# nrsyed/pytorch-yolov3

Hardware: AMD Instinct MI355X
Metric: frames/sec (608x608) (higher is better)
Workload: dtype bf16

## Files before the change

### include/yolov3_hip.h

```cpp
#ifndef YOLOV3_HIP_H
#define YOLOV3_HIP_H

#include <stddef.h>
#include <stdint.h>

#ifdef __cplusplus
extern "C" {
#endif

#define Y3_ABI_VERSION 6

#define Y3_OK 0
#define Y3_ERR_INVALID (-1)
#define Y3_ERR_HIP (-2)
#define Y3_ERR_NODEVICE (-3)

#define Y3_F32 0
#define Y3_BF16 1
#define Y3_F16 2
#define Y3_F64 3

#define Y3_OP_CONV 1
#define Y3_OP_MAXPOOL 2
#define Y3_OP_UPSAMPLE 3
// ... 28 lines not shown
  const float *d_bias;
  int32_t n_anchor, n_attr;
  float anchor_w[8], anchor_h[8];
  int32_t row_offset, rows_total;
  float net_w, net_h;
  float *d_bbox;
  float *d_prob;
  int64_t *d_cls;
  int32_t block_idx;
  int32_t reserved;
  const void *d_weight_frag;
} y3_op;

typedef struct y3_plan y3_plan;

#define Y3_AM_HALO_WIDE 0x0001u
#define Y3_AM_IGEMM3_MID 0x0002u
#define Y3_AM_HALO_NARROW 0x0004u
#define Y3_AM_IGEMM3_1X1_DEEP 0x0008u
#define Y3_AM_HALO_MID 0x0010u
#define Y3_AM_IGEMM3_NARROW 0x0020u
#define Y3_AM_IGEMM3_1X1_BM64 0x0040u
#define Y3_AM_PATCH_WIDE 0x0080u
#define Y3_AM_HALO_TILE256 0x0200u
#define Y3_AM_NO_BN_SHRINK 0x0400u
#define Y3_AM_NO_SMALL_GRID 0x0800u
#define Y3_AM_NO_WRES 0x1000u
#define Y3_AM_HALO_DW 0x4000u
#define Y3_AM_HALO_DW_ALWAYS 0x8000u
#define Y3_AM_1X1_DW 0x10000u
#define Y3_AM_SMALL_DW 0x20000u
#define Y3_AM_SMALL_DW_ALWAYS 0x40000u
#define Y3_AM_SMALL_DW_WIDE 0x80000u
#define Y3_AM_WRES_ALWAYS 0x2000u
#define Y3_AM_DEFAULT (Y3_AM_HALO_WIDE | Y3_AM_HALO_NARROW | Y3_AM_IGEMM3_1X1_DEEP | Y3_AM_HALO_MID | Y3_AM_PATCH_WIDE | Y3_AM_HALO_DW | Y3_AM_1X1_DW | Y3_AM_SMALL_DW | Y3_AM_SMALL_DW_WIDE)
#define Y3_AM_IGEMM_ONLY 0u

typedef struct y3_options {
  int32_t auto_mask, unused0, igemm_version, igemm_ns, igemm_bm;
  int32_t use_graph, fuse_stem, fuse_head, fuse_spp, decode_lanes;
  int32_t fuse_block;
  int32_t reserved[5];
} y3_options;

int y3_abi_version(void);
const char *y3_last_error(void);
int y3_device_count(void);

int y3_plan_create(const y3_op *ops, int n_ops, const void *d_zero, y3_plan **out_plan);
int y3_plan_create_ex(const y3_op *ops, int n_ops, const void *d_zero, const y3_options *options, y3_plan **out_plan);
void y3_options_default(y3_options *options);
void y3_plan_destroy(y3_plan *plan);
int y3_plan_run(y3_plan *plan, const void *d_input, void *stream);
int y3_plan_run_timed(y3_plan *plan, const void *d_input, void *stream, float *ms_per_op);
int y3_plan_run_profiled(y3_plan *plan, const void *d_input, void *stream, float *kernel_ms_per_op);
const char *y3_plan_op_kernel(const y3_plan *plan, int op_index);
double y3_plan_op_flops(const y3_plan *plan, int op_index);
double y3_plan_op_bytes(const y3_plan *plan, int op_index);

int y3_conv_path(const y3_op *op);

size_t y3_conv_fragment_weight_bytes(const y3_op *op, const y3_options *options);
int y3_conv_make_fragment_weights(const y3_op *op, void *d_dst, void *stream);

int y3_set_tuning(const char *key, int value);

int y3_op_run(const y3_op *op, const void *d_input, const void *d_zero, void *stream);

// ... 32 lines not shown
```

### pytorch-yolov3_amd/csrc/api.hip

```cpp
#include <stdarg.h>
#include <string.h>

#include <atomic>
#include <new>
#include <vector>

#include "common.h"

static_assert(sizeof(y3_op) == 248, "y3_op layout is part of the ABI (ctypes mirror in yolov3/_hip.py)");

namespace {
thread_local char g_err[512] = "";
}

static y3_options g_y3_defaults = { (int32_t)Y3_AM_DEFAULT,  0,  2,  2,
                                    0,  0,  1,  1,  1,
                                    4,  0, {0, 0, 0, 0, 0}};
static thread_local const y3_options *tl_y3_opt = nullptr;
const y3_options &y3_opt() { return tl_y3_opt ? *tl_y3_opt : g_y3_defaults; }
static thread_local Y3KernelTimer *tl_y3_timer = nullptr;
Y3KernelTimer *y3_kernel_timer() { return tl_y3_timer; }
#if defined(Y3_X_NOEPI) || defined(Y3_X_S2BOUND) || defined(Y3_X_DEBUG) || defined(Y3_STAMPS)
#define Y3_HAS_DEBUG_KEY 1
static int g_y3_debug = 0;
// ... 75 lines not shown
            const unsigned am = (unsigned)y3_opt().auto_mask;
            const int w = op.in_w;
            const bool k3 = op.ksize == 3 && op.stride == 1 && op.in_c >= 128 && op.out_c >= 128 && !(op.flags & Y3_F_OUT_F32);
            const bool halo_ok = k3 && y3_conv_halo_ws_fits(op);
            bool want_halo = false, want_ws = false;
            if (k3 && w > 64) want_halo = am & Y3_AM_HALO_WIDE;
            else if (k3 && w > 32) { want_halo = am & Y3_AM_HALO_MID; want_ws = am & Y3_AM_IGEMM3_MID; }
            else if (k3) { want_halo = am & Y3_AM_HALO_NARROW; want_ws = am & Y3_AM_IGEMM3_NARROW; }
            else if (op.ksize == 1 && op.in_c >= 1024 && op.out_c >= 128 && !(op.flags & Y3_F_OUT_F32))
              want_ws = (am & Y3_AM_IGEMM3_1X1_DEEP) &&
                        ((am & Y3_AM_NO_SMALL_GRID) || (long long)y3_ceil_div(op.batch * op.out_h * op.out_w, 128) * y3_ceil_div(op.out_c, 128) >= y3_device_cus() / 4);
            if ((am & Y3_AM_1X1_DW) && y3_conv1x1_dw_pays(op))
              return y3_launch_conv1x1_dw(op, in, d_zero, s, name, dry_run, frag_w ? frag_w : op.d_weight_frag);
            const bool small_dw = (am & (Y3_AM_SMALL_DW | Y3_AM_SMALL_DW_ALWAYS)) && !(am & Y3_AM_NO_SMALL_GRID);
            if (small_dw && (y3_conv_dw48_fits(op) || (op.ksize == 3 && y3_conv_dw48_fits_wide(op))))
              return y3_launch_conv_dw48(op, in, d_zero, s, name, dry_run, frag_w ? frag_w : op.d_weight_frag);
            if (!(am & Y3_AM_NO_WRES) && y3_conv1x1_wres_supported(op) && ((am & Y3_AM_WRES_ALWAYS) || y3_conv1x1_wres_pays(op)))
              return y3_launch_conv1x1_wres(op, in, d_zero, s, name, dry_run);
            if (small_dw && op.ksize == 1 && y3_conv_dw48_fits_wide(op))
              return y3_launch_conv_dw48(op, in, d_zero, s, name, dry_run, frag_w ? frag_w : op.d_weight_frag);
            if ((am & Y3_AM_IGEMM3_1X1_BM64) && op.ksize == 1 && op.in_c >= 256 && op.out_c >= 128 && !(op.flags & Y3_F_OUT_F32) &&
                y3_is16(op.dtype))
              return y3_launch_conv_igemm(op, in, d_zero, s, name, dry_run, 3, 3, 64);
            if ((am & Y3_AM_PATCH_WIDE) && op.ksize == 3 && op.stride == 1 && w > 128 && op.out_c >= 128 && y3_conv_patch_fits(op))
              return y3_launch_conv_patch(op, in, d_zero, s, name, dry_run);
            const long long halo_tiles = (long long)y3_ceil_div(op.batch * op.in_h * op.in_w, 192) * (op.out_c / 128);
            const bool small_grid = !(am & Y3_AM_NO_SMALL_GRID) && k3 && halo_tiles < (3 * y3_device_cus()) / 4;
            if (k3 && !small_grid && halo_ok && (((am & Y3_AM_HALO_DW) && y3_conv_halo_dw_pays(op)) ||
                                                 ((am & Y3_AM_HALO_DW_ALWAYS) && y3_conv_halo_dw_fits(op))))
              return y3_launch_conv_halo_dw(op, in, d_zero, s, name, dry_run, frag_w ? frag_w : op.d_weight_frag);
            if (small_grid && y3_is16(op.dtype)) return y3_launch_conv_igemm(op, in, d_zero, s, name, dry_run, 3, 3);
            if (want_halo && halo_ok && !small_grid) return y3_launch_conv_halo(op, in, d_zero, s, name, dry_run);
            if (want_ws) return y3_launch_conv_igemm(op, in, d_zero, s, name, dry_run, 3, 3);
            if (!(am & Y3_AM_NO_SMALL_GRID) && op.ksize == 3 && op.stride == 2 && op.out_c >= 128 && y3_is16(op.dtype) && !(op.flags & Y3_F_OUT_F32) &&
                ((op.in_c == 256 && (long long)op.batch * op.out_h * op.out_w >= 16384) ||
                 (op.in_c == 64 && (long long)op.batch * op.out_h * op.out_w <= 49152)))
              return y3_launch_conv_igemm(op, in, d_zero, s, name, dry_run, 3, 3);
          }
          return y3_launch_conv_igemm(op, in, d_zero, s, name, dry_run);
        }
        case 1: return y3_launch_conv_small(op, in, s, name, dry_run);
        case 3: return y3_launch_conv_stem_mfma(op, in, s, name, dry_run);
        default: return y3_launch_conv_direct(op, in, s, name, dry_run);
      }
    }
    case Y3_OP_MAXPOOL: return y3_launch_maxpool(op, in, s, name, dry_run);
    case Y3_OP_UPSAMPLE: return y3_launch_upsample(op, in, s, name, dry_run);
    case Y3_OP_ADD: return y3_launch_add(op, in, s, name, dry_run);
    case Y3_OP_COPY: return y3_launch_copy(op, in, s, name, dry_run);
    case Y3_OP_YOLO: return y3_launch_yolo(op, in, s, name, dry_run);
    default: break;
  }
  y3_set_error("op for block %d: unknown kind %d", op.block_idx, op.kind);
  return Y3_ERR_INVALID;
}

int run_op(y3_plan *plan, size_t i, const void *d_input, hipStream_t s, const char **name) {
  if (plan->fuse[i] == 2) return Y3_OK;
  if (plan->fuse[i] == 3) return y3_launch_conv_fused_resblock(plan->ops[i], plan->ops[i + 1], s, name, false);
  if (plan->fuse[i] == 6) return y3_launch_conv_block_fused(plan->ops[i], plan->ops[i + 1], s, name, false);
  if (plan->fuse[i] == 4) return y3_launch_conv_head_decode(plan->ops[i], plan->ops[i + 1], plan->d_zero, s, name, false, plan->frag_w[i]);
  if (plan->fuse[i] == 5) return y3_launch_maxpool_spp(plan->ops[i], plan->ops[i + 1], plan->ops[i + 2], s, name, false);
  if (plan->fuse[i] == 1) {
    const y3_op &op0 = plan->ops[i];
    const void *in = (op0.flags & Y3_F_PLAN_INPUT) ? d_input : op0.d_in;
    Y3_REQUIRE(in != nullptr, "op for block %d has no input pointer", op0.block_idx);
    return y3_launch_conv_fused_stem_s2(op0, plan->ops[i + 1], in, s, name, false);
  }
  return dispatch(plan->ops[i], d_input, plan->d_zero, s, name, false, plan->frag_w[i]);
}

bool uses_fragment_weights(const char *kernel) {
  return strncmp(kernel, "conv_halo_dw_", 13) == 0 || strncmp(kernel, "conv1x1_dw_", 11) == 0 || strncmp(kernel, "conv_dw48_", 10) == 0 ||
         strncmp(kernel, "conv_head_decode_dw_", 20) == 0;
}

int make_private_fragment_weights(y3_plan *p, size_t i) {
  const y3_op &op = p->ops[i];
  int prev = -1, owner = -1;
  Y3_HIP_CHECK(hipGetDevice(&prev));
  hipPointerAttribute_t attr;
  if (op.d_weight && hipPointerGetAttributes(&attr, op.d_weight) == hipSuccess) owner = attr.device;
  else (void)hipGetLastError();
  if (owner >= 0 && owner != prev) Y3_HIP_CHECK(hipSetDevice(owner));
  int rc = Y3_OK;
  void *w = nullptr;
  hipStream_t s = nullptr;
  do {
    if (hipMalloc(&w, y3_conv_halo_dw_weight_bytes(op)) != hipSuccess) {
      (void)hipGetLastError();
      y3_set_error("y3_plan_create: no memory for the fragment-order weights of block %d", op.block_idx);
      rc = Y3_ERR_HIP;
      break;
    }
    p->frag_w[i] = w;
    p->frag_own[i] = 1;
    if (hipStreamCreateWithFlags(&s, hipStreamNonBlocking) != hipSuccess) { s = nullptr; rc = Y3_ERR_HIP; }
    if (rc == Y3_OK) rc = y3_conv_halo_dw_make_weights(op, w, s);
    if (rc == Y3_OK && hipStreamSynchronize(s) != hipSuccess) rc = Y3_ERR_HIP;
    if (rc == Y3_ERR_HIP) y3_set_error("y3_plan_create: fragment-order weights of block %d: %s", op.block_idx, hipGetErrorString(hipGetLastError()));
  } while (0);
  if (s) (void)hipStreamDestroy(s);
  if (owner >= 0 && owner != prev) (void)hipSetDevice(prev);
  return rc;
}

}
// ... 2 lines not shown

int y3_abi_version(void) { return Y3_ABI_VERSION; }

const char *y3_last_error(void) { return g_err; }

int y3_device_count(void) {
  int n = 0;
  if (hipGetDeviceCount(&n) != hipSuccess) return 0;
  int ok = 0;
  for (int i = 0; i < n; ++i) {
    hipDeviceProp_t prop;
    if (hipGetDeviceProperties(&prop, i) == hipSuccess && strncmp(prop.gcnArchName, "gfx950", 6) == 0) ++ok;
  }
  return ok;
}

int y3_conv_path(const y3_op *op) {
  if (!op || op->kind != Y3_OP_CONV) return -1;
  return conv_path(*op);
}

size_t y3_conv_fragment_weight_bytes(const y3_op *op, const y3_options *options) {
  if (!op || op->kind != Y3_OP_CONV || conv_path(*op) != 0) return 0;
  y3_options o = options ? *options : g_y3_defaults;
  OptScope scope(&o);
  const char *name = "";
  if (y3_opt().fuse_head && y3_conv_head_dw_fits(*op)) return y3_conv_halo_dw_weight_bytes(*op);
  if (dispatch(*op, nullptr, nullptr, nullptr, &name, true) != Y3_OK) return 0;
  return uses_fragment_weights(name) ? y3_conv_halo_dw_weight_bytes(*op) : 0;
}

int y3_conv_make_fragment_weights(const y3_op *op, void *d_dst, void *stream) {
  Y3_REQUIRE(op && d_dst && op->d_weight, "y3_conv_make_fragment_weights: bad arguments");
  Y3_REQUIRE(y3_conv_halo_dw_fits(*op) || y3_conv1x1_dw_pays(*op) || y3_conv_dw48_fits(*op) || y3_conv_dw48_fits_wide(*op) || y3_conv_head_dw_fits(*op),
             "conv block %d: not a layer of a direct-weights kernel", op->block_idx);
  return y3_conv_halo_dw_make_weights(*op, d_dst, static_cast<hipStream_t>(stream));
}

void y3_options_default(y3_options *options) {
  if (options) *options = g_y3_defaults;
}

int y3_plan_create(const y3_op *ops, int n_ops, const void *d_zero, y3_plan **out_plan) {
  return y3_plan_create_ex(ops, n_ops, d_zero, nullptr, out_plan);
}

int y3_plan_create_ex(const y3_op *ops, int n_ops, const void *d_zero, const y3_options *options, y3_plan **out_plan) {
  Y3_REQUIRE(ops && n_ops > 0 && out_plan, "y3_plan_create: bad arguments");
  Y3_REQUIRE(d_zero, "y3_plan_create: d_zero (zeroed device page) is required");
  y3_plan *p = new (std::nothrow) y3_plan;
  Y3_REQUIRE(p, "y3_plan_create: out of host memory");
  p->opt = options ? *options : g_y3_defaults;
  OptScope scope(&p->opt);
  p->ops.assign(ops, ops + n_ops);
  p->kernel.assign(n_ops, "");
  p->frag_w.assign(n_ops, nullptr);
  p->frag_own.assign(n_ops, 0);
  p->d_zero = d_zero;
  p->fuse.assign(n_ops, 0);
  for (int i = 0; i + 2 < n_ops; ++i)
    if (y3_opt().fuse_spp && y3_maxpool_spp_supported(p->ops[i], p->ops[i + 1], p->ops[i + 2])) {
      p->fuse[i] = 5;
      p->fuse[i + 1] = p->fuse[i + 2] = 2;
    }
  for (int i = 0; i + 1 < n_ops; ++i)
    if (p->fuse[i] != 0) continue;
    else if ((p->ops[i].flags & Y3_F_FUSE_NEXT) && p->ops[i].kind == Y3_OP_CONV &&
        y3_conv_fused_stem_s2_supported(p->ops[i], p->ops[i + 1])) {
// ... 250 lines not shown
```

### pytorch-yolov3_amd/csrc/common.h

```cpp
#pragma once
#include <hip/hip_runtime.h>
#include <hip/hip_ext.h>
#include <stdint.h>
#include <stdio.h>

#include <mutex>

#include "yolov3_hip.h"

typedef __bf16 bf16_t;
typedef float f32x4 __attribute__((ext_vector_type(4)));
typedef float f32x2 __attribute__((ext_vector_type(2)));
typedef __bf16 bf16x8 __attribute__((ext_vector_type(8)));
typedef __bf16 bf16x4 __attribute__((ext_vector_type(4)));
typedef _Float16 f16_t;
typedef _Float16 f16x8 __attribute__((ext_vector_type(8)));
typedef _Float16 f16x4 __attribute__((ext_vector_type(4)));
typedef uint32_t u32x4 __attribute__((ext_vector_type(4)));
typedef uint32_t u32x2 __attribute__((ext_vector_type(2)));

#define Y3_WAVE 64
#ifndef Y3_AUX_W
#define Y3_AUX_W 0
#endif
// ... 64 lines not shown
  }
};

static inline bool y3_is16(int dtype) { return dtype == Y3_BF16 || dtype == Y3_F16; }
static inline int y3_elem_size(int dtype) { return y3_is16(dtype) ? 2 : 4; }
#define Y3_KNAME(dt, pre, post) ((dt) == Y3_BF16 ? pre "bf16" post : ((dt) == Y3_F16 ? pre "f16" post : pre "f32" post))
template <typename F>
static inline int y3_by_dtype(int dtype, F &&f) {
  if (dtype == Y3_BF16) return f(bf16_t{});
  if (dtype == Y3_F16) return f(f16_t{});
  return f(float{});
}
template <typename F>
static inline int y3_by_dtype16(int dtype, F &&f) {
  return dtype == Y3_F16 ? f(f16_t{}) : f(bf16_t{});
}
static inline int y3_ceil_div(int a, int b) { return (a + b - 1) / b; }
static inline void y3_fast_div(uint32_t d, uint32_t &mul, uint32_t &sh) {
  if (d <= 1) { mul = 0; sh = 0; return; }
  sh = 0;
  while ((1u << sh) < d) ++sh;
  mul = (uint32_t)((((uint64_t)1 << 32) * (((uint64_t)1 << sh) - d)) / d + 1);
}

__device__ __forceinline__ int y3_xcd_remap(int bid, int nwg) {
  const int q = nwg >> 3, r = nwg & 7;
  const int xcd = bid & 7, idx = bid >> 3;
  const int base = xcd < r ? xcd * (q + 1) : r * (q + 1) + (xcd - r) * q;
  return base + idx;
}

__host__ __device__ __forceinline__ constexpr int y3_pair_perm(int j) {
  return (j & ~31) | (((j >> 2) & 3) << 3) | (((j >> 4) & 1) << 2) | (j & 3);
}

template <typename T>
__device__ __forceinline__ float y3_to_float(T v);
template <>
__device__ __forceinline__ float y3_to_float<float>(float v) { return v; }
template <>
__device__ __forceinline__ float y3_to_float<bf16_t>(bf16_t v) { return (float)v; }
template <>
__device__ __forceinline__ float y3_to_float<f16_t>(f16_t v) { return (float)v; }

template <typename T>
__device__ __forceinline__ T y3_from_float(float v);
template <>
__device__ __forceinline__ float y3_from_float<float>(float v) { return v; }
template <>
__device__ __forceinline__ bf16_t y3_from_float<bf16_t>(float v) { return (bf16_t)v; }
template <>
__device__ __forceinline__ f16_t y3_from_float<f16_t>(float v) { return (f16_t)v; }

template <typename T>
struct H16;
template <>
struct H16<bf16_t> {
  typedef bf16x8 v8;
  typedef bf16x4 v4;
  static __device__ __forceinline__ f32x4 mfma(const v8 &w, const v8 &x, const f32x4 &acc) {
    return __builtin_amdgcn_mfma_f32_16x16x32_bf16(w, x, acc, 0, 0, 0);
  }
};
template <>
struct H16<f16_t> {
  typedef f16x8 v8;
// ... 153 lines not shown
int y3_launch_conv_fused_stem_s2(const y3_op &op0, const y3_op &op1, const void *d_in, hipStream_t s,
                                 const char **kernel_name, bool dry_run);
bool y3_conv_fused_resblock_supported(const y3_op &op0, const y3_op &op1);
int y3_launch_conv_fused_resblock(const y3_op &op0, const y3_op &op1, hipStream_t s, const char **kernel_name,
                                  bool dry_run);
bool y3_conv_block_fused_supported(const y3_op &op0, const y3_op &op1);
int y3_launch_conv_block_fused(const y3_op &op0, const y3_op &op1, hipStream_t s, const char **kernel_name, bool dry_run);
bool y3_conv_head_decode_supported(const y3_op &op0, const y3_op &op1);
int y3_launch_conv_head_decode(const y3_op &op0, const y3_op &op1, const void *d_zero, hipStream_t s,
                               const char **kernel_name, bool dry_run, const void *frag_w = nullptr);
bool y3_conv_head_dw_fits(const y3_op &op0);
int y3_launch_conv_head_decode_dw(const y3_op &op0, const y3_op &op1, const void *d_zero, hipStream_t s, const char **kernel_name,
                                  bool dry_run, const void *frag_w);
bool y3_conv_halo_ws_fits(const y3_op &op);
bool y3_conv_halo_dw_fits(const y3_op &op);
bool y3_conv_halo_dw_pays(const y3_op &op);
size_t y3_conv_halo_dw_weight_bytes(const y3_op &op);
int y3_conv_halo_dw_make_weights(const y3_op &op, void *dst, hipStream_t s);
int y3_launch_conv_halo_dw(const y3_op &op, const void *d_in, const void *d_zero, hipStream_t s,
                           const char **kernel_name, bool dry_run, const void *frag_w);
int y3_launch_conv_halo(const y3_op &op, const void *d_in, const void *d_zero, hipStream_t s,
                        const char **kernel_name, bool dry_run);
bool y3_conv1x1_wres_supported(const y3_op &op);
bool y3_conv1x1_wres_pays(const y3_op &op);
int y3_launch_conv1x1_wres(const y3_op &op, const void *d_in, const void *d_zero, hipStream_t s, const char **kernel_name,
                           bool dry_run);
bool y3_conv1x1_dw_pays(const y3_op &op);
int y3_launch_conv1x1_dw(const y3_op &op, const void *d_in, const void *d_zero, hipStream_t s, const char **kernel_name,
                         bool dry_run, const void *frag_w);
bool y3_conv_dw48_fits(const y3_op &op);
bool y3_conv_dw48_fits_wide(const y3_op &op);
int y3_launch_conv_dw48(const y3_op &op, const void *d_in, const void *d_zero, hipStream_t s, const char **kernel_name,
                        bool dry_run, const void *frag_w);
bool y3_conv_patch_fits(const y3_op &op);
int y3_launch_conv_patch(const y3_op &op, const void *d_in, const void *d_zero, hipStream_t s,
                         const char **kernel_name, bool dry_run);
const y3_options &y3_opt();
bool y3_conv_igemm_supported(const y3_op &op);
```

### pytorch-yolov3_amd/csrc/conv_dw48.hip

```cpp
#include <utility>

#include "common.h"

namespace {

typedef __attribute__((address_space(3))) void lds_void;
typedef const __attribute__((address_space(1))) void gbl_void;

struct Dw48Args {
  const char *in;
  const char *wgt;
  const float *scale;
  const float *bias;
  const char *res;
  char *out;
  const char *zero;
  int M, H, W, HW, in_ld, out_ld, res_ld, k_ld;
  int in_h, in_w;
  int n_ctiles;
  int nwc;
  int m_tiles;
  int m_inner;
  int hr;
  uint32_t mul_hw, sh_hw, mul_w, sh_w;
// ... 25 lines not shown
  constexpr int SWZ = NKT == 1 ? 7 : 15;
  static_assert((ST == 1 && NH == 1) || (ST == 2 && KS == 3), "stride 2 and channel halves: the 3x3 form only");
  constexpr int BM = 48, MI = 3, NI = 2;
  constexpr int TAPS = KS * KS;
  constexpr int RB = NKT * 128;
  constexpr int S = NKT * TAPS * 2;
  constexpr int DEPTH = S < Y3_DW48_DEPTH ? S : Y3_DW48_DEPTH;
  extern __shared__ __attribute__((aligned(16))) char smem[];

  const int tid = threadIdx.x;
  const int lane = tid & 63;
  const int wave = __builtin_amdgcn_readfirstlane(tid >> 6);
  const int nwaves = blockDim.x >> 6;
  const int fr = lane & 15, fq = lane >> 4;
  const int tile = y3_xcd_remap(blockIdx.x, gridDim.x);
  const int mt = p.m_inner ? tile % p.m_tiles : tile / p.n_ctiles;
  const int ct = p.m_inner ? tile / p.m_tiles : tile % p.n_ctiles;
  const int m0 = mt * BM;
  const int n0 = (ct * p.nwc + wave) * 32;

  const long long q0 = (long long)m0 - (KS == 3 ? p.W + 1 : 0);
  const int pieces = ((p.hr + 1) * RB + 1023) >> 10;
  auto stage = [&](int h) {
    for (int i = wave; i < pieces; i += nwaves) {
      const int o = i * 1024 + lane * 16;
      const int r = o / RB, cpos = (o - r * RB) >> 4;
      const int c = cpos ^ (r & SWZ);
      long long q;
      bool ok;
      if constexpr (ST == 1) {
        q = q0 + r;
        ok = r < p.hr && q >= 0 && q < p.M;
      } else {
        const int e1 = 48, e2 = 97, e3 = 145 + p.W;
        const int pr = r >= e2 ? 1 : 0, pc = ((r >= e1 && r < e2) || r >= e3) ? 1 : 0;
        const int base = r < e1 ? 0 : (r < e2 ? e1 + 1 : (r < e3 ? e2 + p.W : e3 + p.W + 1));
        const long long mm = (long long)m0 + r - base;
        ok = r < p.hr && mm >= 0 && mm < p.M;
        const uint32_t um = ok ? (uint32_t)mm : 0u;
        const uint32_t img = (__umulhi(um, p.mul_hw) + um) >> p.sh_hw;
        const uint32_t rem = um - img * (uint32_t)p.HW;
        const uint32_t oy = (__umulhi(rem, p.mul_w) + rem) >> p.sh_w;
        const uint32_t ox = rem - oy * (uint32_t)p.W;
        q = ((long long)img * p.in_h + 2 * oy + pr) * p.in_w + 2 * ox + pc;
      }
      const char *src = ok ? p.in + (q * p.in_ld) * 2 + h * RB + c * 16 : p.zero;
      __builtin_amdgcn_global_load_lds((gbl_void *)src, (lds_void *)(smem + i * 1024), 16, 0, 0);
    }
  };

  const uint32_t kblocks = (uint32_t)p.k_ld / 32u;
  const uint32_t w_lane = (uint32_t)lane * 16;
  const char *wb[NI];
#pragma unroll
  for (int ni = 0; ni < NI; ++ni) wb[ni] = p.wgt + (((long long)(n0 / 16 + ni) * kblocks) << 10);
  u32x4 wf[DEPTH][NI];
  uint32_t w_img = w_lane;
  if (wave >= p.nwc) {
#pragma unroll 1
    for (int h = 0; h < NH; ++h) {
      if (h > 0) __builtin_amdgcn_s_barrier();
      stage(h);
      asm volatile("s_waitcnt vmcnt(0)" ::: "memory");
      __builtin_amdgcn_s_barrier();
    }
    return;
  }
  stage(0);
  asm volatile("" ::: "memory");
  auto load_w = [&](auto sc, u32x4 (&w)[NI]) {
    constexpr int s = decltype(sc)::value;
    constexpr int kt = s / (2 * TAPS), tap = (s / 2) % TAPS, kh = s & 1;
    const uint32_t voff = w_img + (uint32_t)((tap * (NH * NKT * 2) + kt * 2 + kh) << 10);
    const char *b0 = wb[0], *b1 = wb[1];
    asm volatile("global_load_dwordx4 %0, %1, %2" : "=v"(w[0]) : "v"(voff), "s"(b0));
    asm volatile("global_load_dwordx4 %0, %1, %2" : "=v"(w[1]) : "v"(voff), "s"(b1));
  };
  dw48_for<DEPTH>([&](auto sc) { load_w(sc, wf[decltype(sc)::value]); });

  typedef const __attribute__((address_space(3))) u32x4 lds_u32x4;
  const int lds0 = (int)(size_t)(lds_void *)smem;
  const int zrow = lds0 + p.hr * RB;
  int abase[TAPS][MI], fk4[TAPS];
  {
    uint32_t tapmask[MI];
#pragma unroll
    for (int mi = 0; mi < MI; ++mi) {
      tapmask[mi] = 0x1FFu;
      if constexpr (KS == 3) {
        const uint32_t m = (uint32_t)(m0 + mi * 16 + fr);
        const uint32_t img = (__umulhi(m, p.mul_hw) + m) >> p.sh_hw;
        const uint32_t rem = m - img * (uint32_t)p.HW;
        const uint32_t oy = (__umulhi(rem, p.mul_w) + rem) >> p.sh_w;
        const uint32_t ox = rem - oy * (uint32_t)p.W;
        const uint32_t vx = (ox >= 1u ? 1u : 0u) | 2u | (ST == 2 || ox + 1u < (uint32_t)p.W ? 4u : 0u);
        tapmask[mi] = (oy >= 1u ? vx : 0u) | (vx << 3) | (ST == 2 || oy + 1u < (uint32_t)p.H ? vx << 6 : 0u);
      }
    }
#pragma unroll
    for (int tap = 0; tap < TAPS; ++tap) {
      int r0 = fr + (KS == 3 ? (tap / 3) * p.W + tap % 3 : 0);
      if constexpr (ST == 2) {
        const int ky = tap / 3, kx = tap % 3;
        r0 = fr + (ky == 1 ? (kx == 1 ? 0 : 48) : (kx == 1 ? 97 : 145 + p.W)) + (kx == 2 ? 1 : 0) + (ky == 2 ? p.W : 0);
      }
      fk4[tap] = (fq ^ (r0 & SWZ)) << 4;
#pragma unroll
      for (int mi = 0; mi < MI; ++mi)
        abase[tap][mi] = ((tapmask[mi] >> tap) & 1u) ? lds0 + (mi * 16 + r0) * RB : zrow;
    }
  }

  f32x4 acc[MI][NI];
#pragma unroll
  for (int mi = 0; mi < MI; ++mi)
#pragma unroll
    for (int ni = 0; ni < NI; ++ni) acc[mi][ni] = f32x4{0.f, 0.f, 0.f, 0.f};

  u32x4 xf[3][MI];
  auto read_x = [&](auto sc, u32x4 (&x)[MI]) {
    constexpr int s = decltype(sc)::value;
    constexpr int kt = s / (2 * TAPS), tap = (s / 2) % TAPS, kh = s & 1;
    const int off = ((kt * 8 + kh * 4) << 4) ^ fk4[tap];
#pragma unroll
    for (int mi = 0; mi < MI; ++mi) x[mi] = *reinterpret_cast<lds_u32x4 *>(abase[tap][mi] + off);
  };
  auto mma = [&](const u32x4 (&x)[MI], const u32x4 (&w)[NI]) {
#pragma unroll
    for (int mi = 0; mi < MI; ++mi)
#pragma unroll
      for (int ni = 0; ni < NI; ++ni) acc[mi][ni] = y3_mfma16<T>(w[ni], x[mi], acc[mi][ni]);
  };
  auto run_image = [&]() {
    asm volatile("s_waitcnt vmcnt(%0)" ::"n"(2 * (DEPTH - 1)) : "memory");
    __builtin_amdgcn_s_barrier();
    read_x(HalfC<0>{}, xf[0]);
    if constexpr (S > 1) read_x(HalfC<1>{}, xf[1]);
// ... 202 lines not shown
```

### pytorch-yolov3_amd/yolov3/_hip.py

```python
import ctypes
import os

import torch


_RUNTIME_DEFAULT_QUEUES = 4


def hw_queues():
    try:
        return int(os.environ.get("GPU_MAX_HW_QUEUES") or _RUNTIME_DEFAULT_QUEUES), True
    except ValueError:
        return _RUNTIME_DEFAULT_QUEUES, False

_HERE = os.path.dirname(os.path.abspath(__file__))
LIB_PATH = os.environ.get("Y3_HIP_LIB") or os.path.join(_HERE, "..", "lib", "libyolov3_hip.so")

Y3_F32, Y3_BF16, Y3_F16, Y3_F64 = 0, 1, 2, 3
OP_CONV, OP_MAXPOOL, OP_UPSAMPLE, OP_ADD, OP_COPY, OP_YOLO = 1, 2, 3, 4, 5, 6
F_LEAKY, F_RESIDUAL, F_OUT_F32, F_IN_NCHW_F32, F_IN_NHWC_U8BGR, F_PLAN_INPUT, F_FUSE_NEXT = 1, 2, 4, 8, 16, 32, 64
PATH_IGEMM, PATH_STEM, PATH_DIRECT, PATH_STEM_MFMA = 0, 1, 2, 3


class Y3Op(ctypes.Structure):
    _fields_ = [
        ("kind", ctypes.c_int32), ("dtype", ctypes.c_int32), ("flags", ctypes.c_uint32),
        ("batch", ctypes.c_int32),
        ("in_h", ctypes.c_int32), ("in_w", ctypes.c_int32), ("in_c", ctypes.c_int32), ("in_ld", ctypes.c_int32),
        ("out_h", ctypes.c_int32), ("out_w", ctypes.c_int32), ("out_c", ctypes.c_int32), ("out_ld", ctypes.c_int32),
        ("ksize", ctypes.c_int32), ("stride", ctypes.c_int32), ("pad", ctypes.c_int32),
        ("res_ld", ctypes.c_int32), ("k_ld", ctypes.c_int32), ("cout_pad", ctypes.c_int32),
        ("d_in", ctypes.c_void_p), ("d_out", ctypes.c_void_p), ("d_res", ctypes.c_void_p),
        ("d_weight", ctypes.c_void_p), ("d_scale", ctypes.c_void_p), ("d_bias", ctypes.c_void_p),
        ("n_anchor", ctypes.c_int32), ("n_attr", ctypes.c_int32),
        ("anchor_w", ctypes.c_float * 8), ("anchor_h", ctypes.c_float * 8),
        ("row_offset", ctypes.c_int32), ("rows_total", ctypes.c_int32),
        ("net_w", ctypes.c_float), ("net_h", ctypes.c_float),
        ("d_bbox", ctypes.c_void_p), ("d_prob", ctypes.c_void_p), ("d_cls", ctypes.c_void_p),
        ("block_idx", ctypes.c_int32), ("reserved", ctypes.c_int32),
        ("d_weight_frag", ctypes.c_void_p),
    ]


class Y3Options(ctypes.Structure):
    _fields_ = [(name, ctypes.c_int32) for name in (
        "auto_mask", "unused0", "igemm_version", "igemm_ns", "igemm_bm", "use_graph", "fuse_stem", "fuse_head",
        "fuse_spp", "decode_lanes", "fuse_block")] + [("reserved", ctypes.c_int32 * 5)]


AM_HALO_WIDE, AM_IGEMM3_MID, AM_HALO_NARROW, AM_IGEMM3_1X1_DEEP = 0x0001, 0x0002, 0x0004, 0x0008
AM_HALO_MID, AM_IGEMM3_NARROW, AM_IGEMM3_1X1_BM64, AM_PATCH_WIDE = 0x0010, 0x0020, 0x0040, 0x0080
AM_HALO_TILE256, AM_NO_BN_SHRINK, AM_NO_SMALL_GRID, AM_NO_WRES, AM_WRES_ALWAYS = 0x0200, 0x0400, 0x0800, 0x1000, 0x2000
AM_HALO_DW, AM_HALO_DW_ALWAYS = 0x4000, 0x8000
AM_1X1_DW = 0x10000
AM_SMALL_DW_ALWAYS = 0x40000
AM_SMALL_DW = 0x20000
AM_SMALL_DW_WIDE = 0x80000
AM_DEFAULT = (AM_HALO_WIDE | AM_HALO_NARROW | AM_IGEMM3_1X1_DEEP | AM_HALO_MID | AM_PATCH_WIDE | AM_HALO_DW | AM_1X1_DW | AM_SMALL_DW |
              AM_SMALL_DW_WIDE)
AM_IGEMM_ONLY = 0
AM_HALO_ALL = AM_HALO_WIDE | AM_HALO_NARROW | AM_HALO_MID

ABI_VERSION = 6
_lib = None

PROTOTYPES = {
    "y3_abi_version": (ctypes.c_int, []),
    "y3_last_error": (ctypes.c_char_p, []),
    "y3_device_count": (ctypes.c_int, []),
    "y3_plan_create": (ctypes.c_int, [ctypes.POINTER(Y3Op), ctypes.c_int, ctypes.c_void_p,
                                      ctypes.POINTER(ctypes.c_void_p)]),
    "y3_plan_create_ex": (ctypes.c_int, [ctypes.POINTER(Y3Op), ctypes.c_int, ctypes.c_void_p, ctypes.POINTER(Y3Options),
                                         ctypes.POINTER(ctypes.c_void_p)]),
    "y3_options_default": (None, [ctypes.POINTER(Y3Options)]),
    "y3_plan_destroy": (None, [ctypes.c_void_p]),
    "y3_plan_run": (ctypes.c_int, [ctypes.c_void_p, ctypes.c_void_p, ctypes.c_void_p]),
    "y3_plan_run_timed": (ctypes.c_int, [ctypes.c_void_p, ctypes.c_void_p, ctypes.c_void_p,
                                         ctypes.POINTER(ctypes.c_float)]),
    "y3_plan_run_profiled": (ctypes.c_int, [ctypes.c_void_p, ctypes.c_void_p, ctypes.c_void_p,
                                            ctypes.POINTER(ctypes.c_float)]),
    "y3_plan_op_kernel": (ctypes.c_char_p, [ctypes.c_void_p, ctypes.c_int]),
    "y3_plan_op_flops": (ctypes.c_double, [ctypes.c_void_p, ctypes.c_int]),
    "y3_plan_op_bytes": (ctypes.c_double, [ctypes.c_void_p, ctypes.c_int]),
    "y3_conv_path": (ctypes.c_int, [ctypes.POINTER(Y3Op)]),
    "y3_conv_fragment_weight_bytes": (ctypes.c_size_t, [ctypes.POINTER(Y3Op), ctypes.POINTER(Y3Options)]),
    "y3_conv_make_fragment_weights": (ctypes.c_int, [ctypes.POINTER(Y3Op), ctypes.c_void_p, ctypes.c_void_p]),
    "y3_set_tuning": (ctypes.c_int, [ctypes.c_char_p, ctypes.c_int]),
    "y3_op_run": (ctypes.c_int, [ctypes.POINTER(Y3Op), ctypes.c_void_p, ctypes.c_void_p, ctypes.c_void_p]),
    "y3_detect_workspace_bytes": (ctypes.c_size_t, [ctypes.c_int, ctypes.c_int]),
    "y3_detect": (ctypes.c_int, [ctypes.c_void_p, ctypes.c_void_p, ctypes.c_void_p, ctypes.c_int, ctypes.c_int,
                                 ctypes.c_void_p, ctypes.c_float, ctypes.c_double, ctypes.c_void_p,
                                 ctypes.c_size_t, ctypes.c_void_p, ctypes.c_void_p, ctypes.c_void_p,
# ... 79 lines not shown
```

Measured before the change: 5823.

## Add stride-2 3x3 direct-weights conv kernel with fragment-order weights

Adds a new conv_s2dw kernel for stride-2 3x3 convolutions. It stages the four parity planes of the input tile in LDS with double buffering and streams pre-permuted fragment-order weights straight into registers through a deep prefetch pipeline. It is enabled by default for layers where the tile count covers most CUs, excluding in_c==256. The shared stride-2 row and tap mapping helpers move into common.h and are reused by dw48. The fragment-weight check is broadened to any 16-bit implicit-GEMM layer, which adds LDS pressure and tuning risk for the new kernel.

Result: no change. 5836 (median of 6 runs) (+0.2%).

```diff
diff --git a/include/yolov3_hip.h b/include/yolov3_hip.h
--- a/include/yolov3_hip.h
+++ b/include/yolov3_hip.h
@@ -84,8 +84,10 @@
 #define Y3_AM_SMALL_DW 0x20000u
 #define Y3_AM_SMALL_DW_ALWAYS 0x40000u
 #define Y3_AM_SMALL_DW_WIDE 0x80000u
+#define Y3_AM_S2_DW 0x100000u
+#define Y3_AM_S2_DW_ALWAYS 0x200000u
 #define Y3_AM_WRES_ALWAYS 0x2000u
-#define Y3_AM_DEFAULT (Y3_AM_HALO_WIDE | Y3_AM_HALO_NARROW | Y3_AM_IGEMM3_1X1_DEEP | Y3_AM_HALO_MID | Y3_AM_PATCH_WIDE | Y3_AM_HALO_DW | Y3_AM_1X1_DW | Y3_AM_SMALL_DW | Y3_AM_SMALL_DW_WIDE)
+#define Y3_AM_DEFAULT (Y3_AM_HALO_WIDE | Y3_AM_HALO_NARROW | Y3_AM_IGEMM3_1X1_DEEP | Y3_AM_HALO_MID | Y3_AM_PATCH_WIDE | Y3_AM_HALO_DW | Y3_AM_1X1_DW | Y3_AM_SMALL_DW | Y3_AM_SMALL_DW_WIDE | Y3_AM_S2_DW)
 #define Y3_AM_IGEMM_ONLY 0u
 
 typedef struct y3_options {
diff --git a/pytorch-yolov3_amd/csrc/api.hip b/pytorch-yolov3_amd/csrc/api.hip
--- a/pytorch-yolov3_amd/csrc/api.hip
+++ b/pytorch-yolov3_amd/csrc/api.hip
@@ -131,6 +131,8 @@
             if (small_grid && y3_is16(op.dtype)) return y3_launch_conv_igemm(op, in, d_zero, s, name, dry_run, 3, 3);
             if (want_halo && halo_ok && !small_grid) return y3_launch_conv_halo(op, in, d_zero, s, name, dry_run);
             if (want_ws) return y3_launch_conv_igemm(op, in, d_zero, s, name, dry_run, 3, 3);
+            if (((am & Y3_AM_S2_DW) && y3_conv_s2dw_pays(op)) || ((am & Y3_AM_S2_DW_ALWAYS) && y3_conv_s2dw_fits(op)))
+              return y3_launch_conv_s2dw(op, in, d_zero, s, name, dry_run, frag_w ? frag_w : op.d_weight_frag);
             if (!(am & Y3_AM_NO_SMALL_GRID) && op.ksize == 3 && op.stride == 2 && op.out_c >= 128 && y3_is16(op.dtype) && !(op.flags & Y3_F_OUT_F32) &&
                 ((op.in_c == 256 && (long long)op.batch * op.out_h * op.out_w >= 16384) ||
                  (op.in_c == 64 && (long long)op.batch * op.out_h * op.out_w <= 49152)))
@@ -171,7 +173,7 @@
 
 bool uses_fragment_weights(const char *kernel) {
   return strncmp(kernel, "conv_halo_dw_", 13) == 0 || strncmp(kernel, "conv1x1_dw_", 11) == 0 || strncmp(kernel, "conv_dw48_", 10) == 0 ||
-         strncmp(kernel, "conv_head_decode_dw_", 20) == 0;
+         strncmp(kernel, "conv_head_decode_dw_", 20) == 0 || strncmp(kernel, "conv_s2dw_", 10) == 0;
 }
 
 int make_private_fragment_weights(y3_plan *p, size_t i) {
@@ -240,8 +242,9 @@
 
 int y3_conv_make_fragment_weights(const y3_op *op, void *d_dst, void *stream) {
   Y3_REQUIRE(op && d_dst && op->d_weight, "y3_conv_make_fragment_weights: bad arguments");
-  Y3_REQUIRE(y3_conv_halo_dw_fits(*op) || y3_conv1x1_dw_pays(*op) || y3_conv_dw48_fits(*op) || y3_conv_dw48_fits_wide(*op) || y3_conv_head_dw_fits(*op),
-             "conv block %d: not a layer of a direct-weights kernel", op->block_idx);
+  Y3_REQUIRE(op->kind == Y3_OP_CONV && y3_is16(op->dtype) && conv_path(*op) == 0 && op->cout_pad % 32 == 0 && op->k_ld % 32 == 0,
+             "conv block %d: no fragment-order layout for this layer (16-bit implicit-GEMM layers, cout_pad and k_ld multiples of 32)",
+             op->block_idx);
   return y3_conv_halo_dw_make_weights(*op, d_dst, static_cast<hipStream_t>(stream));
 }
 
diff --git a/pytorch-yolov3_amd/csrc/common.h b/pytorch-yolov3_amd/csrc/common.h
--- a/pytorch-yolov3_amd/csrc/common.h
+++ b/pytorch-yolov3_amd/csrc/common.h
@@ -120,6 +120,26 @@
 
 __host__ __device__ __forceinline__ constexpr int y3_pair_perm(int j) {
   return (j & ~31) | (((j >> 2) & 3) << 3) | (((j >> 4) & 1) << 2) | (j & 3);
+}
+
+__host__ __device__ __forceinline__ constexpr int y3_s2_rows(int P, int W) { return 4 * P + 2 * W + 2; }
+__host__ __device__ __forceinline__ constexpr int y3_s2_tap_row(int tap, int P, int W) {
+  return (tap / 3 == 1 ? (tap % 3 == 1 ? 0 : P) : (tap % 3 == 1 ? 2 * P + 1 : 3 * P + 1 + W)) + (tap % 3 == 2 ? 1 : 0) +
+         (tap / 3 == 2 ? W : 0);
+}
+__device__ __forceinline__ void y3_s2_row_plane(int r, int P, int W, int &pr, int &pc, int &dm) {
+  const int e1 = P, e2 = 2 * P + 1, e3 = 3 * P + 1 + W;
+  pr = r >= e2 ? 1 : 0;
+  pc = ((r >= e1 && r < e2) || r >= e3) ? 1 : 0;
+  dm = r - (r < e1 ? 0 : (r < e2 ? e1 + 1 : (r < e3 ? e2 + W : e3 + W + 1)));
+}
+__device__ __forceinline__ long long y3_s2_source(uint32_t um, int pr, int pc, int HW, int W, int in_h, int in_w, uint32_t mul_hw,
+                                                  uint32_t sh_hw, uint32_t mul_w, uint32_t sh_w) {
+  const uint32_t img = (__umulhi(um, mul_hw) + um) >> sh_hw;
+  const uint32_t rem = um - img * (uint32_t)HW;
+  const uint32_t oy = (__umulhi(rem, mul_w) + rem) >> sh_w;
+  const uint32_t ox = rem - oy * (uint32_t)W;
+  return ((long long)img * in_h + 2 * oy + pr) * in_w + 2 * ox + pc;
 }
 
 template <typename T>
@@ -339,6 +359,10 @@
 bool y3_conv_dw48_fits_wide(const y3_op &op);
 int y3_launch_conv_dw48(const y3_op &op, const void *d_in, const void *d_zero, hipStream_t s, const char **kernel_name,
                         bool dry_run, const void *frag_w);
+bool y3_conv_s2dw_fits(const y3_op &op);
+bool y3_conv_s2dw_pays(const y3_op &op);
+int y3_launch_conv_s2dw(const y3_op &op, const void *d_in, const void *d_zero, hipStream_t s, const char **kernel_name, bool dry_run,
+                        const void *frag_w);
 bool y3_conv_patch_fits(const y3_op &op);
 int y3_launch_conv_patch(const y3_op &op, const void *d_in, const void *d_zero, hipStream_t s,
                          const char **kernel_name, bool dry_run);
diff --git a/pytorch-yolov3_amd/csrc/conv_dw48.hip b/pytorch-yolov3_amd/csrc/conv_dw48.hip
--- a/pytorch-yolov3_amd/csrc/conv_dw48.hip
+++ b/pytorch-yolov3_amd/csrc/conv_dw48.hip
@@ -81,17 +81,11 @@
         q = q0 + r;
         ok = r < p.hr && q >= 0 && q < p.M;
       } else {
-        const int e1 = 48, e2 = 97, e3 = 145 + p.W;
-        const int pr = r >= e2 ? 1 : 0, pc = ((r >= e1 && r < e2) || r >= e3) ? 1 : 0;
-        const int base = r < e1 ? 0 : (r < e2 ? e1 + 1 : (r < e3 ? e2 + p.W : e3 + p.W + 1));
-        const long long mm = (long long)m0 + r - base;
+        int pr, pc, dm;
+        y3_s2_row_plane(r, BM, p.W, pr, pc, dm);
+        const long long mm = (long long)m0 + dm;
         ok = r < p.hr && mm >= 0 && mm < p.M;
-        const uint32_t um = ok ? (uint32_t)mm : 0u;
-        const uint32_t img = (__umulhi(um, p.mul_hw) + um) >> p.sh_hw;
-        const uint32_t rem = um - img * (uint32_t)p.HW;
-        const uint32_t oy = (__umulhi(rem, p.mul_w) + rem) >> p.sh_w;
-        const uint32_t ox = rem - oy * (uint32_t)p.W;
-        q = ((long long)img * p.in_h + 2 * oy + pr) * p.in_w + 2 * ox + pc;
+        q = y3_s2_source(ok ? (uint32_t)mm : 0u, pr, pc, p.HW, p.W, p.in_h, p.in_w, p.mul_hw, p.sh_hw, p.mul_w, p.sh_w);
       }
       const char *src = ok ? p.in + (q * p.in_ld) * 2 + h * RB + c * 16 : p.zero;
       __builtin_amdgcn_global_load_lds((gbl_void *)src, (lds_void *)(smem + i * 1024), 16, 0, 0);
@@ -150,8 +144,7 @@
     for (int tap = 0; tap < TAPS; ++tap) {
       int r0 = fr + (KS == 3 ? (tap / 3) * p.W + tap % 3 : 0);
       if constexpr (ST == 2) {
-        const int ky = tap / 3, kx = tap % 3;
-        r0 = fr + (ky == 1 ? (kx == 1 ? 0 : 48) : (kx == 1 ? 97 : 145 + p.W)) + (kx == 2 ? 1 : 0) + (ky == 2 ? p.W : 0);
+        r0 = fr + y3_s2_tap_row(tap, BM, p.W);
       }
       fk4[tap] = (fq ^ (r0 & SWZ)) << 4;
 #pragma unroll
diff --git a/pytorch-yolov3_amd/csrc/conv_s2dw.hip b/pytorch-yolov3_amd/csrc/conv_s2dw.hip
--- /dev/null
+++ b/pytorch-yolov3_amd/csrc/conv_s2dw.hip
@@ -0,0 +1,303 @@
+#include <utility>
+
+#include "common.h"
+
+namespace {
+
+typedef __attribute__((address_space(3))) void lds_void;
+typedef const __attribute__((address_space(1))) void gbl_void;
+
+constexpr int S2_P = 96;
+constexpr int S2_BN = 256;
+
+struct S2dwArgs {
+  const char *in;
+  const char *wgt;
+  const float *scale;
+  const float *bias;
+  const char *res;
+  char *out;
+  const char *zero;
+  int M, H, W, HW, in_h, in_w, in_ld, out_ld, res_ld, k_ld;
+  int m_tiles, n_ctiles;
+  int m_inner;
+  int nchunks;
+  int rows;
+  int np;
+  uint32_t mul_hw, sh_hw, mul_w, sh_w;
+  uint32_t flags;
+};
+
+template <int V>
+struct S2C { static constexpr int value = V; };
+template <int... I, typename F>
+__device__ __forceinline__ void s2_for_impl(std::integer_sequence<int, I...>, F &&f) { (f(S2C<I>{}), ...); }
+template <int N, typename F>
+__device__ __forceinline__ void s2_for(F &&f) { s2_for_impl(std::make_integer_sequence<int, N>{}, f); }
+
+template <int N>
+__device__ __forceinline__ void s2_wait_vm(u32x4 (&w)[2]) {
+  asm volatile("s_waitcnt vmcnt(%2)" : "+v"(w[0]), "+v"(w[1]) : "n"(N) : "memory");
+}
+
+template <typename T, int PPW>
+__global__ __launch_bounds__(512) void conv_s2dw_kernel(S2dwArgs p) {
+  static_assert(sizeof(T) == 2, "16-bit storage modes only");
+  constexpr int P = S2_P, MI = 6, NI = 2;
+  constexpr int S = 18;
+  constexpr int DEPTH = 6;
+  static_assert(S % DEPTH == 0 && S % 3 == 0 && PPW <= S - DEPTH, "half-step bookkeeping");
+  extern __shared__ __attribute__((aligned(16))) char smem[];
+
+  const int tid = threadIdx.x;
+  const int lane = tid & 63;
+  const int wave = __builtin_amdgcn_readfirstlane(tid >> 6);
+  const int fr = lane & 15, fq = lane >> 4;
+  const int tile = y3_xcd_remap(blockIdx.x, gridDim.x);
+  const int mt = p.m_inner ? tile % p.m_tiles : tile / p.n_ctiles;
+  const int ct = p.m_inner ? tile / p.m_tiles : tile % p.n_ctiles;
+  const int m0 = mt * P;
+  const int n0 = ct * S2_BN + wave * 32;
+  const int buf = p.np * 1024;
+
+  int soff[PPW];
+#pragma unroll
+  for (int j = 0; j < PPW; ++j) {
+    const int i = j * 8 + wave;
+    const int r = i * 8 + (lane >> 3);
+    const int c = (lane & 7) ^ (r & 7);
+    int pr, pc, dm;
+    y3_s2_row_plane(r, P, p.W, pr, pc, dm);
+    const long long mm = (long long)m0 + dm;
+    const bool ok = i < p.np && r < p.rows && mm >= 0 && mm < p.M;
+    const long long q = y3_s2_source(ok ? (uint32_t)mm : 0u, pr, pc, p.HW, p.W, p.in_h, p.in_w, p.mul_hw, p.sh_hw, p.mul_w, p.sh_w);
+    soff[j] = ok ? (int)(q * p.in_ld * 2 + c * 16) : -1;
+  }
+  auto piece = [&](int j, int chunk) {
+    const int i = j * 8 + wave;
+    const char *src = soff[j] >= 0 ? p.in + soff[j] + chunk * 128 : p.zero;
+    char *dst = i < p.np ? smem + (chunk & 1) * buf + i * 1024 : smem + 2 * buf;
+    __builtin_amdgcn_global_load_lds((gbl_void *)src, (lds_void *)dst, 16, 0, 0);
+  };
+
+  const uint32_t kblocks = (uint32_t)p.k_ld / 32u;
+  const uint32_t cb = 2u * (uint32_t)p.nchunks;
+  const uint32_t w_lane = (uint32_t)lane * 16;
+  const char *wb[NI];
+#pragma unroll
+  for (int ni = 0; ni < NI; ++ni) wb[ni] = p.wgt + (((long long)(n0 / 16 + ni) * kblocks) << 10);
+  u32x4 wf[DEPTH][NI];
+  auto load_w = [&](auto sc, uint32_t wc, u32x4 (&w)[NI]) {
+    constexpr int s = decltype(sc)::value, tap = s / 2, kh = s & 1;
+    const uint32_t voff = wc + (((uint32_t)tap * cb + kh) << 10);
+    const char *b0 = wb[0], *b1 = wb[1];
+    asm volatile("global_load_dwordx4 %0, %1, %2" : "=v"(w[0]) : "v"(voff), "s"(b0));
+    asm volatile("global_load_dwordx4 %0, %1, %2" : "=v"(w[1]) : "v"(voff), "s"(b1));
+  };
+
+  if (wave == 0) __builtin_amdgcn_global_load_lds((gbl_void *)p.zero, (lds_void *)(smem + 2 * buf), 16, 0, 0);
+#pragma unroll
+  for (int j = 0; j < PPW; ++j) piece(j, 0);
+  asm volatile("" ::: "memory");
+  s2_for<DEPTH>([&](auto sc) { load_w(sc, w_lane, wf[decltype(sc)::value]); });
+
+  typedef const __attribute__((address_space(3))) u32x4 lds_u32x4;
+  const int lds0 = (int)(size_t)(lds_void *)smem;
+  const int zaddr = lds0 + 2 * buf;
+  int toff[9];
+#pragma unroll
+  for (int t = 0; t < 9; ++t) {
+    const int r0 = fr + y3_s2_tap_row(t, P, p.W);
+    toff[t] = (r0 << 7) + ((fq ^ (r0 & 7)) << 4);
+  }
+  unsigned long long mk_top[MI], mk_left[MI];
+#pragma unroll
+  for (int mi = 0; mi < MI; ++mi) {
+    const uint32_t m = (uint32_t)(m0 + mi * 16 + fr);
+    const uint32_t img = (__umulhi(m, p.mul_hw) + m) >> p.sh_hw;
+    const uint32_t rem = m - img * (uint32_t)p.HW;
+    const uint32_t oy = (__umulhi(rem, p.mul_w) + rem) >> p.sh_w;
+    const uint32_t ox = rem - oy * (uint32_t)p.W;
+    mk_top[mi] = __builtin_amdgcn_ballot_w64(oy >= 1u);
+    mk_left[mi] = __builtin_amdgcn_ballot_w64(ox >= 1u);
+  }
+
+  f32x4 acc[MI][NI];
+#pragma unroll
+  for (int mi = 0; mi < MI; ++mi)
+#pragma unroll
+    for (int ni = 0; ni < NI; ++ni) acc[mi][ni] = f32x4{0.f, 0.f, 0.f, 0.f};
+
+  u32x4 xf[3][MI];
+  auto read_x = [&](auto sc, int base, u32x4 (&x)[MI]) {
+    constexpr int s = decltype(sc)::value, tap = s / 2, kh = s & 1, ky = tap / 3, kx = tap % 3;
+    int a = (base + toff[tap]) ^ (kh << 6);
+    asm volatile("" : "+v"(a));
+#pragma unroll
+    for (int mi = 0; mi < MI; ++mi) {
+      int off = a + mi * 2048;
+      if constexpr (ky == 0 || kx == 0) {
+        unsigned long long ok = ky == 0 ? mk_top[mi] : ~0ull;
+        if constexpr (kx == 0) ok &= mk_left[mi];
+        const int real = off;
+        asm("v_cndmask_b32_e64 %0, %1, %2, %3" : "=v"(off) : "v"(zaddr), "v"(real), "s"(ok));
+      }
+      x[mi] = *reinterpret_cast<lds_u32x4 *>(off);
+    }
+  };
+  auto mma = [&](const u32x4 (&x)[MI], const u32x4 (&w)[NI]) {
+#pragma unroll
+    for (int mi = 0; mi < MI; ++mi)
+#pragma unroll
+      for (int ni = 0; ni < NI; ++ni) acc[mi][ni] = y3_mfma16<T>(w[ni], x[mi], acc[mi][ni]);
+  };
+
+  auto run_chunk = [&](auto lastc, int c) {
+    constexpr bool LAST = decltype(lastc)::value;
+    const int cur = lds0 + (c & 1) * buf;
+    const uint32_t wc = w_lane + ((uint32_t)(2 * c) << 10);
+    s2_for<S>([&](auto sc) {
+      constexpr int s = decltype(sc)::value, slot = s % DEPTH;
+      constexpr int yw = LAST ? 2 * ((s + DEPTH < S ? s + DEPTH : S) - s - 1) : 2 * (DEPTH - 1);
+      constexpr int lo = s - DEPTH > 0 ? s - DEPTH : 0, hi = s < PPW ? s : PPW;
+      constexpr int yp = LAST ? 0 : (hi > lo ? hi - lo : 0);
+      s2_wait_vm<yw + yp>(wf[slot]);
+      __builtin_amdgcn_sched_barrier(0);
+      if constexpr (s + 2 < S) read_x(S2C<s + 2>{}, cur, xf[(s + 2) % 3]);
+      mma(xf[s % 3], wf[slot]);
+#pragma unroll
+      for (int i = 0; i < MI; ++i) {
+        __builtin_amdgcn_sched_group_barrier(0x100, 1, 0);
+        __builtin_amdgcn_sched_group_barrier(0x008, 2, 0);
+      }
+      __builtin_amdgcn_sched_barrier(0);
+      if constexpr (s + DEPTH < S) load_w(S2C<s + DEPTH>{}, wc, wf[slot]);
+      else if constexpr (!LAST) load_w(S2C<s + DEPTH - S>{}, wc + (2u << 10), wf[slot]);
+      if constexpr (!LAST && s < PPW) piece(s, c + 1);
+    });
+    if constexpr (!LAST) {
+      asm volatile("s_waitcnt vmcnt(%0)" ::"n"(2 * (S - PPW)) : "memory");
+      __builtin_amdgcn_s_barrier();
+      const int nxt = lds0 + ((c + 1) & 1) * buf;
+      read_x(S2C<0>{}, nxt, xf[0]);
+      read_x(S2C<1>{}, nxt, xf[1]);
+    }
+  };
+
+  asm volatile("s_waitcnt vmcnt(%0)" ::"n"(2 * DEPTH) : "memory");
+  __builtin_amdgcn_s_barrier();
+  read_x(S2C<0>{}, lds0, xf[0]);
+  read_x(S2C<1>{}, lds0, xf[1]);
+#pragma unroll 1
+  for (int c = 0; c + 1 < p.nchunks; ++c) {
+#pragma unroll
+    for (int t = 0; t < 9; ++t) asm volatile("" : "+v"(toff[t]));
+    run_chunk(S2C<0>{}, c);
+  }
+  run_chunk(S2C<1>{}, p.nchunks - 1);
+
+  const int co = n0 + fq * 8;
+  const f32x4 sc_lo = *reinterpret_cast<const f32x4 *>(p.scale + co), sc_hi = *reinterpret_cast<const f32x4 *>(p.scale + co + 4);
+  const f32x4 bi_lo = *reinterpret_cast<const f32x4 *>(p.bias + co), bi_hi = *reinterpret_cast<const f32x4 *>(p.bias + co + 4);
+  const bool leaky = p.flags & Y3_F_LEAKY;
+  const bool has_res = p.flags & Y3_F_RESIDUAL;
+  u32x4 resv[MI];
+  if (has_res) {
+#pragma unroll
+    for (int mi = 0; mi < MI; ++mi) {
+      const int m = m0 + mi * 16 + fr;
+      resv[mi] = m < p.M ? *reinterpret_cast<const u32x4 *>(p.res + ((long long)m * p.res_ld + co) * 2) : u32x4{0u, 0u, 0u, 0u};
+    }
+  }
+#pragma unroll
+  for (int mi = 0; mi < MI; ++mi) {
+    const int m = m0 + mi * 16 + fr;
+    float v[8];
+    y3_bn_leaky8(v, acc[mi][0], acc[mi][1], sc_lo, sc_hi, bi_lo, bi_hi, leaky);
+    if (has_res) y3_add8<T>(v, resv[mi]);
+    if (m < p.M) *reinterpret_cast<u32x4 *>(p.out + ((long long)m * p.out_ld + co) * 2) = y3_pack8<T>(v);
+  }
+}
+
+int s2dw_pieces(int W) {
+  const int np = (y3_s2_rows(S2_P, W) + 7) / 8;
+  return (2 * np + 1) * 1024 <= 160 * 1024 ? np : 0;
+}
+
+}
+
+bool y3_conv_s2dw_fits(const y3_op &op) {
+  if (op.kind != Y3_OP_CONV || !y3_is16(op.dtype)) return false;
+  if (op.ksize != 3 || op.pad != 1 || op.stride != 2 || op.in_h % 2 != 0 || op.in_w % 2 != 0) return false;
+  if (op.flags & (Y3_F_OUT_F32 | Y3_F_IN_NCHW_F32 | Y3_F_IN_NHWC_U8BGR | Y3_F_PLAN_INPUT)) return false;
+  if (op.in_c % 64 != 0 || op.out_c % S2_BN != 0 || op.cout_pad < op.out_c || op.cout_pad % 32 != 0) return false;
+  if (op.in_ld % 8 != 0 || op.out_ld % 8 != 0 || op.k_ld % 32 != 0 || op.k_ld < 9 * op.in_c) return false;
+  if ((op.flags & Y3_F_RESIDUAL) && op.res_ld % 8 != 0) return false;
+  if (s2dw_pieces(op.out_w) == 0) return false;
+  if ((long long)op.batch * op.in_h * op.in_w * op.in_ld * 2 >= (1ll << 31)) return false;
+  return true;
+}
+
+bool y3_conv_s2dw_pays(const y3_op &op) {
+  if (!y3_conv_s2dw_fits(op) || op.in_c == 256) return false;
+  const long long tiles = (long long)y3_ceil_div(op.batch * op.out_h * op.out_w, S2_P) * (op.out_c / S2_BN);
+  return tiles >= (long long)y3_device_cus() * 3 / 4;
+}
+
+int y3_launch_conv_s2dw(const y3_op &op, const void *d_in, const void *d_zero, hipStream_t s, const char **kernel_name, bool dry_run,
+                        const void *frag_w) {
+  Y3_REQUIRE(y3_conv_s2dw_fits(op), "conv block %d: not a shape for the stride-2 direct-weights kernel", op.block_idx);
+  *kernel_name = Y3_KNAME(op.dtype, "conv_s2dw_", "_96x256");
+  if (dry_run) return Y3_OK;
+  void *tmp = nullptr;
+  if (!frag_w) {
+    Y3_HIP_CHECK(hipMallocAsync(&tmp, y3_conv_halo_dw_weight_bytes(op), s));
+    const int rc = y3_conv_halo_dw_make_weights(op, tmp, s);
+    if (rc != Y3_OK) { (void)hipFreeAsync(tmp, s); return rc; }
+    frag_w = tmp;
+  }
+  S2dwArgs a;
+  a.in = static_cast<const char *>(d_in);
+  a.wgt = static_cast<const char *>(frag_w);
+  a.scale = op.d_scale; a.bias = op.d_bias;
+  a.res = static_cast<const char *>(op.d_res);
+  a.out = static_cast<char *>(op.d_out);
+  a.zero = static_cast<const char *>(d_zero);
+  a.H = op.out_h; a.W = op.out_w; a.HW = op.out_h * op.out_w;
+  a.in_h = op.in_h; a.in_w = op.in_w;
+  a.M = op.batch * a.HW;
+  a.in_ld = op.in_ld; a.out_ld = op.out_ld; a.res_ld = op.res_ld; a.k_ld = op.k_ld;
+  a.m_tiles = y3_ceil_div(a.M, S2_P);
+  a.n_ctiles = op.out_c / S2_BN;
+  a.m_inner = 9.0 * op.in_c * op.out_c > (double)op.batch * op.in_h * op.in_w * op.in_c;
+  a.nchunks = op.in_c / 64;
+  a.rows = y3_s2_rows(S2_P, a.W);
+  a.np = s2dw_pieces(a.W);
+  y3_fast_div((uint32_t)a.HW, a.mul_hw, a.sh_hw);
+  y3_fast_div((uint32_t)a.W, a.mul_w, a.sh_w);
+  a.flags = op.flags;
+  const int ppw = (a.np + 7) / 8;
+  const size_t lds = (size_t)(2 * a.np + 1) * 1024;
+  const dim3 grid(a.m_tiles * a.n_ctiles), block(512);
+  const int rc = y3_by_dtype16(op.dtype, [&](auto tag) {
+    typedef decltype(tag) T;
+    static Y3DeviceOnce once;
+    {
+      const int rc1 = once.run([]() -> int {
+#define Y3_S2DW_ATTR(PPW_) Y3_HIP_CHECK(hipFuncSetAttribute(reinterpret_cast<const void *>(conv_s2dw_kernel<T, PPW_>), hipFuncAttributeMaxDynamicSharedMemorySize, 160 * 1024))
+        Y3_S2DW_ATTR(7); Y3_S2DW_ATTR(8); Y3_S2DW_ATTR(9); Y3_S2DW_ATTR(10);
+#undef Y3_S2DW_ATTR
+        return Y3_OK;
+      });
+      if (rc1 != Y3_OK) return rc1;
+    }
+    if (ppw <= 7) Y3_LAUNCH((conv_s2dw_kernel<T, 7>), grid, block, lds, s, a);
+    else if (ppw == 8) Y3_LAUNCH((conv_s2dw_kernel<T, 8>), grid, block, lds, s, a);
+    else if (ppw == 9) Y3_LAUNCH((conv_s2dw_kernel<T, 9>), grid, block, lds, s, a);
+    else Y3_LAUNCH((conv_s2dw_kernel<T, 10>), grid, block, lds, s, a);
+    Y3_HIP_CHECK(hipGetLastError());
+    return Y3_OK;
+  });
+  if (tmp) (void)hipFreeAsync(tmp, s);
+  return rc;
+}
diff --git a/pytorch-yolov3_amd/yolov3/_hip.py b/pytorch-yolov3_amd/yolov3/_hip.py
--- a/pytorch-yolov3_amd/yolov3/_hip.py
+++ b/pytorch-yolov3_amd/yolov3/_hip.py
@@ -56,8 +56,9 @@
 AM_SMALL_DW_ALWAYS = 0x40000
 AM_SMALL_DW = 0x20000
 AM_SMALL_DW_WIDE = 0x80000
+AM_S2_DW, AM_S2_DW_ALWAYS = 0x100000, 0x200000
 AM_DEFAULT = (AM_HALO_WIDE | AM_HALO_NARROW | AM_IGEMM3_1X1_DEEP | AM_HALO_MID | AM_PATCH_WIDE | AM_HALO_DW | AM_1X1_DW | AM_SMALL_DW |
-              AM_SMALL_DW_WIDE)
+              AM_SMALL_DW_WIDE | AM_S2_DW)
 AM_IGEMM_ONLY = 0
 AM_HALO_ALL = AM_HALO_WIDE | AM_HALO_NARROW | AM_HALO_MID
 
```
